# francescofugazzi/3dgsconverter

Hardware: NVIDIA H100
Metric: Msplats/s SOR k=16 (higher is better)
Workload: dtype f32

## Files before the change

### 3dgsconverter_b200/csrc/gsx_abi.cu

```cuda
#include "../../include/gsx.h"

#include "gsx_common.cuh"
#include "gsx_compact.cuh"
#include "gsx_compressed_ply.cuh"
#include "gsx_density.cuh"
#include "gsx_hostcopy.cuh"
#include "gsx_hostrows.cuh"
#include "gsx_kmeans.cuh"
#include "gsx_knn_exact.cuh"
#include "gsx_masks.cuh"
#include "gsx_morton.cuh"
#include "gsx_ply.cuh"
#include "gsx_radix.cuh"
#include "gsx_readers.cuh"
#include "gsx_records.cuh"
#include "gsx_sog.cuh"
#include "gsx_sog_decode.cuh"
#include "gsx_sor.cuh"
#include "gsx_splat_codecs.cuh"

#include <atomic>
#include <math.h>
#include <stdarg.h>
#include <stdio.h>
// ... 166 lines not shown
int gsx_sor_build_from_sorted(const float* spos4_dev, const uint8_t* flags_dev, int64_t n, const float* bmin_host,
                              float cell, void* ws, int64_t ws_bytes, void* stream) {
    SorWs w;
    int rc = carve_grid_checked(ws, ws_bytes, n, w);
    if (rc) return rc;
    GSX_REQUIRE(cell > 0.f, GSX_ERR_ARG, "sor: cell size must be > 0");
    return sor_build_from_sorted((const float4*)spos4_dev, flags_dev, n, bmin_host, cell, w, (cudaStream_t)stream);
}

int gsx_sor_mean_dists_range(int64_t n, int64_t q_begin, int64_t q_end, int32_t k, int32_t hash_mode,
                             const float* bmin_host, float cell, void* ws, int64_t ws_bytes, float* final_means_dev,
                             unsigned long long* stats_dev, void* stream) {
    SorWs w;
    int rc = carve_grid_checked(ws, ws_bytes, n, w);
    if (rc) return rc;
    return sor_mean_dists(w, q_begin, q_end, 1, 0, k, hash_mode, bmin_host, cell, final_means_dev, stats_dev,
                          (cudaStream_t)stream);
}

int gsx_sor_mean_dists_strided(int64_t n, int32_t stride, int32_t phase, int32_t k, int32_t hash_mode,
                               const float* bmin_host, float cell, void* ws, int64_t ws_bytes, float* final_means_dev,
                               unsigned long long* stats_dev, void* stream) {
    SorWs w;
    int rc = carve_grid_checked(ws, ws_bytes, n, w);
    if (rc) return rc;
    return sor_mean_dists(w, 0, n, stride, phase, k, hash_mode, bmin_host, cell, final_means_dev, stats_dev,
                          (cudaStream_t)stream);
}

int gsx_sor_mean_dists(int64_t n, int32_t k, int32_t hash_mode, const float* bmin_host, float cell, void* ws,
                       int64_t ws_bytes, float* final_means_dev, unsigned long long* stats_dev, void* stream) {
    return gsx_sor_mean_dists_range(n, 0, n, k, hash_mode, bmin_host, cell, ws, ws_bytes, final_means_dev, stats_dev,
                                    stream);
}

int64_t gsx_mean_std_workspace_bytes(int64_t n) { return (int64_t)mean_std_ws_bytes(n); }

int gsx_mean_std_f32(const float* a_dev, int64_t n, float* out_dev, void* ws, int64_t ws_bytes, void* stream) {
    return mean_std_f32(a_dev, n, out_dev, ws, (size_t)ws_bytes, (cudaStream_t)stream);
}

int64_t gsx_pairwise_slots(int64_t n) { return pairwise_slots(n); }

int gsx_pairwise_leaves_dist(const float* a_local_dev, int64_t base, int64_t n_local, int64_t n_global, int32_t sq,
                             const float* meanstd_dev, const float* halo_dev, const int64_t* bases_dev, int32_t world,
                             float* slot_dev, void* stream) {
    return pairwise_leaves_dist(a_local_dev, base, n_local, n_global, sq, meanstd_dev, halo_dev,
                                (const long long*)bases_dev, world, slot_dev, (cudaStream_t)stream);
}

int gsx_pairwise_finish(float* slot_dev, int64_t n_global, int32_t sq, float* meanstd_dev, void* stream) {
    GSX_REQUIRE(n_global >= 1, GSX_ERR_ARG, "pairwise_finish: n must be >= 1");
    return pairwise_finish(slot_dev, n_global, sq, meanstd_dev, (cudaStream_t)stream);
}

int gsx_threshold_mask(const float* a_dev, int64_t n, const float* meanstd_dev, float threshold_factor,
                       uint8_t* mask_dev, void* stream) {
    return threshold_mask(a_dev, n, meanstd_dev, threshold_factor, mask_dev, (cudaStream_t)stream);
}

int gsx_sor_filter_device(const float* xyz_dev, int64_t n, int32_t k, float threshold_factor, int32_t hash_mode,
                          uint8_t* mask_dev, float* means_dev, void* ws, int64_t ws_bytes, void* stream) {
    cudaStream_t st = (cudaStream_t)stream;
    SorWs w;
    int rc = carve_checked(ws, ws_bytes, n, w);
    if (rc) return rc;
// ... 419 lines not shown
```

### 3dgsconverter_b200/csrc/gsx_sor.cu

```cuda
#include "gsx_common.cuh"
#include "gsx_sor.cuh"

#include "gsx_radix.cuh"
#include <math.h>

namespace gsx {

#define GSX_D2LIM_BITS 0x60ad78ebu
#define GSX_FULL 0xffffffffu

constexpr int kCellCodeBits = 15;
constexpr float kCellCodeScale = (float)(1 << (kCellCodeBits / 3));
constexpr float kCellCodeMax = kCellCodeScale - 1.f;
constexpr int kSmallBucket = 64;
constexpr int kQueryBatch = 16;
constexpr int kMergeThreshold = 9;
constexpr int kKnnMinBlocks = 8;
constexpr int kFlatSupers = 8;
const char* sor_build_info() {
    return "knn=r02c;epi_smem=1;first_sort=1;query_batch=16;minblocks=8;merge_threshold=9;small_bucket=64;"
           "flat_supers=8;knn16=0;tma=0;i32=1;cell_order=hilbert15";
}


SorWs sor_carve(void* ws, int64_t ws_bytes, int64_t n, size_t sort_ws_bytes) {
    SorWs w;
    Carver c(ws, (size_t)ws_bytes);
    int64_t nchunk = (n + 31) / 32, nsuper = (nchunk + 31) / 32;
    w.n = n;
    w.spos = c.take<float4>(n);
    w.tab_se = c.take<int2>(n);
    w.tab_box = c.take<float4>(2 * n);
    w.startbits = c.take<uint32_t>(nchunk);
    w.cellbits = c.take<uint32_t>(nchunk);
    w.bigbits = c.take<uint32_t>(nchunk);
    w.startlist = c.take<uint32_t>(n / 8 + 1024);
    w.caabb = c.take<float4>(2 * nchunk);
    w.saabb = c.take<float4>(2 * nsuper);
    w.partial = c.take<float>(6 * 1024);
    w.minmax = c.take<float>(8);
    w.counters = c.take<unsigned int>(64);
    w.stats = c.take<unsigned long long>(8);
    w.meanstd = c.take<float>(8);
    w.ms_bytes = mean_std_ws_bytes(n);
    w.ms_ws = c.take<char>(w.ms_bytes);
    w.grid_total = align_up(c.off, 256);
    w.keys0 = c.take<uint64_t>(n);
    w.keys1 = c.take<uint64_t>(n);
    w.sort_ws_bytes = sort_ws_bytes;
    w.sort_ws = c.take<char>(sort_ws_bytes);
    w.total = align_up(c.off, 256);
    w.ok = c.ok();
    w.grid_ok = w.grid_total <= (size_t)(ws_bytes > 0 ? ws_bytes : 0);
// ... 729 lines not shown
    const unsigned tail_blocks = (sl.capacity + 255) / 256;
    k_sor_bucket_tail<<<tail_blocks, 256, 0, st>>>(w.spos, flags, n, bmin[0], bmin[1], bmin[2], cell, M64, w.tab_se,
                                                   w.tab_box, w.bigbits, sl);
    GSX_KERNEL_CHECK();
    k_sor_big_buckets<<<sm_count() * 8, 256, 0, st>>>(w.bigbits, w.startbits, w.spos, w.caabb, n, bmin[0], bmin[1], bmin[2],
                                                      cell, M64, w.tab_se, w.tab_box, sl);
    GSX_KERNEL_CHECK();
    const int resident = sm_count() * 2;
    k_sor_finish_gated<<<resident, 1024, 0, st>>>(w.spos, n, bmin[0], bmin[1], bmin[2], cell, M64, w.tab_se, w.startbits,
                                                  w.cellbits, w.caabb, w.saabb, sl.count + 1);
    GSX_KERNEL_CHECK();
    k_sor_bucket_boxes_gated<<<resident * 4, 256, 0, st>>>(w.startbits, w.spos, w.caabb, w.tab_se, n, bmin[0], bmin[1],
                                                           bmin[2], cell, M64, w.tab_box, sl.count + 1);
    GSX_KERNEL_CHECK();
    return GSX_OK;
}


__device__ __forceinline__ uint32_t probe_hash(int nx, int ny, int nz, uint32_t n, uint64_t M, int mode) {
    if (mode == GSX_HASH_MODE_I32WRAP) {
        int32_t h = (int32_t)((uint32_t)nx * 73856093u) ^ (int32_t)((uint32_t)ny * 19349663u) ^
                    (int32_t)((uint32_t)nz * 83492791u);
        uint32_t a = h < 0 ? (uint32_t)(-(int64_t)h) : (uint32_t)h;
        uint32_t r = fastmod_u32(a, M, n);
        return h < 0 ? (r ? n - r : 0u) : r;
    } else {
        int64_t h = ((int64_t)nx * 73856093LL) ^ ((int64_t)ny * 19349663LL) ^ ((int64_t)nz * 83492791LL);
        int64_t r = h % (int64_t)n;
        if (r < 0) r += n;
        return (uint32_t)r;
    }
}

__device__ __forceinline__ float box_lb(const float4* __restrict__ aabb, int64_t id, float qx, float qy, float qz) {
    float4 a = __ldg(aabb + 2 * id), b = __ldg(aabb + 2 * id + 1);
    float dx = fmaxf(fmaxf(__fsub_rn(a.x, qx), __fsub_rn(qx, a.w)), 0.f);
    float dy = fmaxf(fmaxf(__fsub_rn(a.y, qy), __fsub_rn(qy, b.x)), 0.f);
    float dz = fmaxf(fmaxf(__fsub_rn(a.z, qz), __fsub_rn(qz, b.y)), 0.f);
    return __fadd_rn(__fadd_rn(__fmul_rn(dx, dx), __fmul_rn(dy, dy)), __fmul_rn(dz, dz));
}

__device__ __forceinline__ float cmpx(float v, int j, bool take_min) {
    float o = __shfl_xor_sync(GSX_FULL, v, j);
    return take_min ? fminf(v, o) : fmaxf(v, o);
}

__device__ __forceinline__ float warp_sort32(float v, int lane) {
#pragma unroll
    for (int k = 2; k <= 32; k <<= 1) {
#pragma unroll
        for (int j = k >> 1; j > 0; j >>= 1) v = cmpx(v, j, ((lane & k) == 0) == ((lane & j) == 0));
    }
    return v;
}

template <int NREG>
struct TopK {
    float v0, v1;
    float tau;
    int K;
    __device__ __forceinline__ void init(int k) {
        K = k;
        v0 = v1 = tau = __uint_as_float(GSX_D2LIM_BITS);
    }
    __device__ __forceinline__ void refresh_tau() {
        tau = (NREG == 2 && K > 32) ? __shfl_sync(GSX_FULL, v1, K - 33) : __shfl_sync(GSX_FULL, v0, K - 1);
    }
    __device__ __forceinline__ void insert(float x, int lane) {
        float up0 = __shfl_up_sync(GSX_FULL, v0, 1);
        if (NREG == 2) {
            float top0 = __shfl_sync(GSX_FULL, v0, 31);
            float up1 = __shfl_up_sync(GSX_FULL, v1, 1);
            if (lane == 0) up1 = top0;
            if (v1 > x) v1 = fmaxf(up1, x);
        }
        if (lane == 0) up0 = 0.f;
        if (v0 > x) v0 = fmaxf(up0, x);
        refresh_tau();
    }
    __device__ __forceinline__ void merge32(float nv, int lane) {
        nv = warp_sort32(nv, lane);
        if (__all_sync(GSX_FULL, v0 == __uint_as_float(GSX_D2LIM_BITS))) {
            v0 = nv;
            refresh_tau();
            return;
        }
        float r = __shfl_sync(GSX_FULL, nv, 31 - lane);
        float m = fminf(v0, r);
#pragma unroll
        for (int j = 16; j > 0; j >>= 1) m = cmpx(m, j, (lane & j) == 0);
        v0 = m;
        refresh_tau();
    }
};

typedef int pos_t;

template <int NREG, bool STATS>
__device__ __forceinline__ void scan32(const float4* __restrict__ spos, pos_t j, bool valid, float qx, float qy,
                                       float qz, TopK<NREG>& tk, int lane, unsigned long long& n_scanned) {
    float d2 = INFINITY;
    if (valid) {
        float4 c = __ldg(spos + j);
        float ax = __fsub_rn(qx, c.x), ay = __fsub_rn(qy, c.y), az = __fsub_rn(qz, c.z);
        d2 = __fadd_rn(__fadd_rn(__fmul_rn(ax, ax), __fmul_rn(ay, ay)), __fmul_rn(az, az));
    }
    if (STATS) n_scanned += __popc(__ballot_sync(GSX_FULL, valid));
    bool pass = valid && d2 > 1.0e-12f && d2 < tk.tau;
    unsigned m = __ballot_sync(GSX_FULL, pass);
    if (NREG == 1 && __popc(m) >= kMergeThreshold) {
        tk.merge32(pass ? d2 : __uint_as_float(GSX_D2LIM_BITS), lane);
        return;
    }
    while (m) {
        int src = __ffs(m) - 1;
        m &= m - 1;
        float x = __shfl_sync(GSX_FULL, d2, src);
        if (x < tk.tau) tk.insert(x, lane);
    }
}

template <int NREG, bool STATS, int ES>
__global__ void __launch_bounds__(256, kKnnMinBlocks)
    k_sor_knn(const float4* __restrict__ spos, const int2* __restrict__ tab_se, const float4* __restrict__ tab_box,
              const uint32_t* __restrict__ cellbits, const float4* __restrict__ caabb,
              const float4* __restrict__ saabb, float* __restrict__ final_means, unsigned int* __restrict__ work,
              int64_t q_begin, int64_t q_end, int q_stride, int q_phase, int K, int hash_mode, float bx, float by,
              float bz, float cell,
              uint32_t n, uint64_t M, unsigned long long* __restrict__ stats) {
    const int lane = lane_id();
    unsigned long long st_visits = 0, st_scanned = 0, st_boxes = 0, st_queries = 0;
    static_assert(ES >= 0 && ES <= 33, "a row holds at most the 32 ranks of one register + the row number");
    extern __shared__ float s_epi[];
    float* const epi = s_epi + (threadIdx.x >> 5) * (kQueryBatch * (ES > 0 ? ES : 1));
    const int pdx = lane / 9 - 1, pdy = (lane / 3) % 3 - 1, pdz = lane % 3 - 1;

    for (;;) {
        unsigned int b0 = 0;
        if (lane == 0) b0 = atomicAdd(work, (unsigned)kQueryBatch);
        b0 = __shfl_sync(GSX_FULL, b0, 0);
        int64_t qb = q_begin + ((int64_t)(b0 / kQueryBatch) * q_stride + q_phase) * kQueryBatch;
        if (qb >= q_end) break;
        int64_t qe = qb + kQueryBatch < q_end ? qb + kQueryBatch : q_end;
        const uint32_t cellword = __ldg(cellbits + (qb >> 5));
        int ps = 0, pc = 0;
        float blx = 0.f, bly = 0.f, blz = 0.f, bhx = 0.f, bhy = 0.f, bhz = 0.f;
        const pos_t qb_p = (pos_t)qb, qe_p = (pos_t)qe;
#pragma unroll 1
        for (pos_t i = qb_p; i < qe_p; ++i) {
            const float4 q = __ldg(spos + i);
            const uint32_t w_i = (i >> 5) == (qb_p >> 5) ? cellword : __ldg(cellbits + (i >> 5));
            if (i == qb_p || ((w_i >> (i & 31)) & 1u)) {
                const int gx = (int)floorf(__fdiv_rn(__fsub_rn(q.x, bx), cell));
                const int gy = (int)floorf(__fdiv_rn(__fsub_rn(q.y, by), cell));
                const int gz = (int)floorf(__fdiv_rn(__fsub_rn(q.z, bz), cell));
                ps = 0, pc = 0;
                if (lane < 27) {
                    uint32_t h = probe_hash(gx + pdx, gy + pdy, gz + pdz, n, M, hash_mode);
                    const int2 se = __ldg(tab_se + h);
                    ps = se.x;
                    pc = se.y - se.x;
                    if (pc > 0) {
                        const float4 b0 = __ldg(tab_box + 2 * (size_t)h), b1 = __ldg(tab_box + 2 * (size_t)h + 1);
                        blx = b0.x, bly = b0.y, blz = b0.z, bhx = b1.x, bhy = b1.y, bhz = b1.z;
                    }
                }
            }
            if (STATS) {
                int tot = pc;
#pragma unroll
                for (int o = 16; o > 0; o >>= 1) tot += __shfl_xor_sync(GSX_FULL, tot, o);
                st_visits += (unsigned long long)tot;
                st_queries += 1;
            }
            TopK<NREG> tk;
            tk.init(K);

            unsigned pkey = 0xffffffffu;
            if (pc > 0) {
                float dx = fmaxf(fmaxf(__fsub_rn(blx, q.x), __fsub_rn(q.x, bhx)), 0.f);
                float dy = fmaxf(fmaxf(__fsub_rn(bly, q.y), __fsub_rn(q.y, bhy)), 0.f);
                float dz = fmaxf(fmaxf(__fsub_rn(blz, q.z), __fsub_rn(q.z, bhz)), 0.f);
                pkey = __float_as_uint(__fadd_rn(__fadd_rn(__fmul_rn(dx, dx), __fmul_rn(dy, dy)), __fmul_rn(dz, dz)));
            }

            int skip_chunk = -1;
            {
                int s13 = __shfl_sync(GSX_FULL, ps, 13), c13 = __shfl_sync(GSX_FULL, pc, 13);
                if (c13 > kSmallBucket && i >= s13 && i < (pos_t)s13 + c13) {
                    skip_chunk = (int)(i >> 5);
                    const pos_t j = ((pos_t)skip_chunk << 5) + lane;
                    scan32<NREG, STATS>(spos, j, j >= s13 && j < (pos_t)s13 + c13, q.x, q.y, q.z, tk, lane,
                                        st_scanned);
                }
            }

#pragma unroll 1
            for (;;) {
                const unsigned mp = __reduce_min_sync(GSX_FULL, pkey);
                if (mp == 0xffffffffu || !(__uint_as_float(mp) < tk.tau)) break;
                const int p = __ffs(__ballot_sync(GSX_FULL, pkey == mp)) - 1;
                if (lane == p) pkey = 0xffffffffu;
                const int s = __shfl_sync(GSX_FULL, ps, p), c = __shfl_sync(GSX_FULL, pc, p);
                const pos_t e = (pos_t)s + c;
                if (c <= kSmallBucket) {
#pragma unroll 1
                    for (pos_t base = s; base < e; base += 32)
                        scan32<NREG, STATS>(spos, base + lane, base + lane < e, q.x, q.y, q.z, tk, lane, st_scanned);
                    continue;
                }
                const int skip = p == 13 ? skip_chunk : -1;
                const int fc = s >> 5, lc = (int)((e - 1) >> 5);
                const int fs = fc >> 5, ls = lc >> 5;
                auto chunk_group = [&](const int cbase) {
                    const int cid = cbase + lane;
                    const bool cv = cid >= fc && cid <= lc && cid != skip;
                    unsigned ckey = 0xffffffffu;
                    if (cv) {
                        float lb = box_lb(caabb, cid, q.x, q.y, q.z);
                        if (lb < tk.tau) ckey = __float_as_uint(lb);
                    }
                    if (STATS) st_boxes += __popc(__ballot_sync(GSX_FULL, cv));
                    for (;;) {
                        unsigned mc = __reduce_min_sync(GSX_FULL, ckey);
                        if (mc == 0xffffffffu || !(__uint_as_float(mc) < tk.tau)) break;
                        int srcc = __ffs(__ballot_sync(GSX_FULL, ckey == mc)) - 1;
                        if (lane == srcc) ckey = 0xffffffffu;
                        const pos_t j = ((pos_t)(cbase + srcc) << 5) + lane;
                        scan32<NREG, STATS>(spos, j, j >= s && j < e, q.x, q.y, q.z, tk, lane, st_scanned);
                    }
                };
                if (ls - fs < kFlatSupers) {
                    for (int cb = fc; cb <= lc; cb += 32) chunk_group(cb);
                    continue;
                }
                for (int sb = fs; sb <= ls; sb += 32) {
                    const int sid = sb + lane;
                    unsigned skey = 0xffffffffu;
                    if (sid <= ls) {
                        float lb = box_lb(saabb, sid, q.x, q.y, q.z);
                        if (lb < tk.tau) skey = __float_as_uint(lb);
                    }
                    if (STATS) st_boxes += __popc(__ballot_sync(GSX_FULL, sid <= ls));
                    for (;;) {
                        unsigned ms = __reduce_min_sync(GSX_FULL, skey);
                        if (ms == 0xffffffffu || !(__uint_as_float(ms) < tk.tau)) break;
                        int srcs = __ffs(__ballot_sync(GSX_FULL, skey == ms)) - 1;
                        if (lane == srcs) skey = 0xffffffffu;
                        chunk_group((sb + srcs) * 32);
                    }
                }
            }

            const float d0 = __fsqrt_rn(tk.v0), d1 = NREG == 2 ? __fsqrt_rn(tk.v1) : 0.f;
            if (ES > 0) {
                float* row = epi + (int)(i - qb_p) * ES;
                if (ES <= 32) {
                    if (lane < ES) row[lane] = lane == ES - 1 ? q.w : d0;
                } else {
                    row[lane] = d0;
                    if (lane == 0) row[ES - 1] = q.w;
                }
                continue;
            }
            int valid = __popc(__ballot_sync(GSX_FULL, lane < K && d0 < 0.9e10f));
            if (NREG == 2) valid += __popc(__ballot_sync(GSX_FULL, lane + 32 < K && d1 < 0.9e10f));
            float sum = 0.f;
            for (int r = 0; r < valid; ++r) {
                float x = (NREG == 2 && r >= 32) ? __shfl_sync(GSX_FULL, d1, r - 32) : __shfl_sync(GSX_FULL, d0, r);
                sum = __fadd_rn(sum, x);
            }
            if (lane == 0) final_means[__float_as_int(q.w)] = valid > 0 ? __fdiv_rn(sum, (float)valid) : 0.f;
        }
        if (ES > 0) {
            __syncwarp();
            if (lane < (int)(qe - qb)) {
                const float* row = epi + lane * ES;
                float sum = 0.f;
                int valid = 0;
                for (int r = 0; r < K; ++r) {
                    const float x = row[r];
                    if (x < 0.9e10f) {
                        sum = __fadd_rn(sum, x);
                        ++valid;
                    }
                }
                final_means[__float_as_int(row[ES - 1])] = valid > 0 ? __fdiv_rn(sum, (float)valid) : 0.f;
            }
            __syncwarp();
        }
    }
    if (STATS && lane == 0) {
        atomicAdd(stats + 0, st_visits);
        atomicAdd(stats + 1, st_scanned);
        atomicAdd(stats + 2, st_boxes);
        atomicAdd(stats + 3, st_queries);
    }
}

__global__ void k_fill_f32(float* p, int64_t n, float v) {
    int64_t i = (int64_t)blockIdx.x * blockDim.x + threadIdx.x;
    if (i < n) p[i] = v;
}

template <int NREG, int ES>
static int launch_knn(SorWs& w, int64_t q_begin, int64_t q_end, int q_stride, int q_phase, int K, int hash_mode,
                      const float* bmin, float cell,
                      float* final_means, unsigned long long* stats, uint64_t M, int64_t want, cudaStream_t st) {
    const auto kernel = stats ? k_sor_knn<NREG, true, ES> : k_sor_knn<NREG, false, ES>;
    int per_sm = 0;
    const size_t smem = (size_t)8 * kQueryBatch * ES * sizeof(float);
    GSX_CUDA_CHECK(cudaOccupancyMaxActiveBlocksPerMultiprocessor(&per_sm, kernel, 256, smem));
    int64_t grid = (int64_t)sm_count() * (per_sm > 0 ? per_sm : 4);
    if (grid > want) grid = want;
    if (grid < 1) grid = 1;
    kernel<<<(int)grid, 256, smem, st>>>(w.spos, w.tab_se, w.tab_box, w.cellbits, w.caabb, w.saabb, final_means, w.counters,
                                         q_begin, q_end, q_stride, q_phase, K, hash_mode, bmin[0], bmin[1], bmin[2], cell,
                                         (uint32_t)w.n, M, stats);
    return GSX_OK;
}

int sor_mean_dists(SorWs& w, int64_t q_begin, int64_t q_end, int q_stride, int q_phase, int k, int hash_mode,
                   const float* bmin, float cell,
                   float* final_means, unsigned long long* stats, cudaStream_t st) {
    GSX_NVTX("gsx::sor_mean_dists(k_sor_knn)");
    int64_t n = w.n;
    GSX_REQUIRE(k >= 1, GSX_ERR_ARG, "sor: k must be >= 1 (got %d)", k);
    GSX_REQUIRE(hash_mode == 0 || hash_mode == 1, GSX_ERR_ARG, "sor: bad hash_mode %d", hash_mode);
    GSX_REQUIRE(q_begin >= 0 && q_end <= n && q_begin <= q_end, GSX_ERR_ARG, "sor: bad query range");
    GSX_REQUIRE(q_stride >= 1 && q_phase >= 0 && q_phase < q_stride, GSX_ERR_ARG, "sor: bad query stride/phase");
    int K = k < 50 ? k : 50;
    if (q_end == q_begin) return GSX_OK;
    if (!(cell > 1e-8f)) {
        GSX_REQUIRE(q_begin == 0 && q_end == n, GSX_ERR_UNSUPPORTED, "sor: degenerate cell with a query range");
        k_fill_f32<<<(int)((n + 255) / 256), 256, 0, st>>>(final_means, n, 0.f);
        GSX_KERNEL_CHECK();
        return GSX_OK;
    }
    GSX_CUDA_CHECK(cudaMemsetAsync(w.counters, 0, sizeof(unsigned int), st));
    uint64_t M = 0xFFFFFFFFFFFFFFFFull / (uint64_t)n + 1ull;
    int64_t nq = (q_end - q_begin + q_stride - 1) / q_stride + kQueryBatch;
    int64_t want = (nq + (int64_t)kQueryBatch * 8 - 1) / ((int64_t)kQueryBatch * 8);
    int rc;
    if (K <= 16)
        rc = launch_knn<1, 17>(w, q_begin, q_end, q_stride, q_phase, K, hash_mode, bmin, cell, final_means, stats, M, want, st);
    else if (K <= 32)
        rc = launch_knn<1, 33>(w, q_begin, q_end, q_stride, q_phase, K, hash_mode, bmin, cell, final_means, stats, M, want, st);
    else
        rc = launch_knn<2, 0>(w, q_begin, q_end, q_stride, q_phase, K, hash_mode, bmin, cell, final_means, stats, M, want, st);
    if (rc) return rc;
    GSX_KERNEL_CHECK();
    return GSX_OK;
}

}
```

### 3dgsconverter_b200/gsx/_abi.py

```python
from __future__ import annotations

import ctypes as C
import os
from pathlib import Path

_PKG = Path(__file__).resolve().parent.parent
LIB_PATH = Path(os.environ.get("GSX_LIB", _PKG / "lib" / "libgsx.so"))


class GsxError(RuntimeError):
    """A libgsx entry point returned a non-zero status."""


if not LIB_PATH.exists():
    raise ImportError(
        f"libgsx.so not found at {LIB_PATH}: build it with `python -c 'import __graft_entry__ as g; g.build()'` "
        "(nvcc, sm_90a).  gsx has no CPU fallback.")

lib = C.CDLL(str(LIB_PATH))

_f32p = C.POINTER(C.c_float)
_vp = C.c_void_p
_i64 = C.c_int64
_i32 = C.c_int32

_SIGS = {
    "gsx_last_error": (C.c_char_p, []),
    "gsx_version": (C.c_int, []),
    "gsx_build_info": (C.c_char_p, []),
    "gsx_device_sm_count": (C.c_int, []),
    "gsx_kernel_launches": (C.c_longlong, []),
    "gsx_sor_workspace_bytes": (_i64, [_i64]),
    "gsx_sor_grid_workspace_bytes": (_i64, [_i64]),
    "gsx_sor_minmax": (C.c_int, [_vp, _i64, _vp, _vp, _i64, _vp]),
    "gsx_sor_cell_size": (C.c_float, [_f32p, _i64]),
    "gsx_sor_build": (C.c_int, [_vp, _i64, _f32p, C.c_float, _vp, _i64, _vp]),
    "gsx_sor_dist_local_run": (C.c_int, [_vp, _i64, _i64, _i64, _i32, _f32p, C.c_float, _vp, _vp, _vp, _i64, _vp]),
    "gsx_sor_dist_merge": (C.c_int, [_vp, _i64, _i64, _i64, _i64, _f32p, C.c_float, _vp, _vp, _vp, _i64, _vp]),
    "gsx_sor_spos_offset": (_i64, [_i64]),
    "gsx_sor_build_from_sorted": (C.c_int, [_vp, _vp, _i64, _f32p, C.c_float, _vp, _i64, _vp]),
    "gsx_sor_mean_dists": (C.c_int, [_i64, _i32, _i32, _f32p, C.c_float, _vp, _i64, _vp, _vp, _vp]),
    "gsx_sor_mean_dists_range": (C.c_int, [_i64, _i64, _i64, _i32, _i32, _f32p, C.c_float, _vp, _i64, _vp, _vp, _vp]),
    "gsx_sor_mean_dists_strided": (C.c_int, [_i64, _i32, _i32, _i32, _i32, _f32p, C.c_float, _vp, _i64, _vp, _vp, _vp]),
    "gsx_sort_pairs_workspace_bytes": (_i64, [_i64]),
    "gsx_sort_pairs": (C.c_int, [_vp, _vp, _i64, _i32, _i32, _vp, _i64, _vp]),
    "gsx_mean_std_workspace_bytes": (_i64, [_i64]),
    "gsx_mean_std_f32": (C.c_int, [_vp, _i64, _vp, _vp, _i64, _vp]),
    "gsx_pairwise_slots": (_i64, [_i64]),
    "gsx_pairwise_leaves_dist": (C.c_int, [_vp, _i64, _i64, _i64, _i32, _vp, _vp, _vp, _i32, _vp, _vp]),
    "gsx_pairwise_finish": (C.c_int, [_vp, _i64, _i32, _vp, _vp]),
    "gsx_threshold_mask": (C.c_int, [_vp, _i64, _vp, C.c_float, _vp, _vp]),
    "gsx_sor_filter_device": (C.c_int, [_vp, _i64, _i32, C.c_float, _i32, _vp, _vp, _vp, _i64, _vp]),
    "gsx_sor_filter_host": (C.c_int, [_vp, _i64, _i32, C.c_float, _i32, _vp, _vp]),
    "gsx_knn_exact_workspace_bytes": (_i64, [_i64]),
    "gsx_knn_exact_mean_dists": (C.c_int, [_vp, _i64, _i32, _vp, _vp, _i64, _vp]),
    "gsx_sor_ckdtree_filter_host": (C.c_int, [_vp, _i64, _i32, C.c_float, _vp, _vp]),
    "gsx_bbox_mask": (C.c_int, [_vp, _i64, _f32p, _vp, _vp]),
    "gsx_alpha_mask": (C.c_int, [_vp, _i64, C.c_double, _vp, _vp]),
    "gsx_alpha_logit_threshold": (C.c_double, [C.c_double]),
    "gsx_compact_workspace_bytes": (_i64, [_i64]),
    "gsx_compact_points": (C.c_int, [_vp, _i64, _vp, _vp, _vp, _vp, _vp, _vp, C.POINTER(_i64), _vp, _i64, _vp]),
    "gsx_density_workspace_bytes": (_i64, [_i64, _i64]),
    "gsx_density_voxel_count": (C.c_int, [_vp, _i64, C.c_float, _i64, _vp, _vp, _i64, C.POINTER(_i64),
                                          C.POINTER(_i64), _vp, _i64, _vp]),
    "gsx_density_member_mask": (C.c_int, [_vp, _i64, C.c_float, _vp, _i64, _vp, _vp, _i64, _vp]),
    "gsx_density_voxel_range": (None, [_f32p, C.c_float, C.POINTER(_i64), C.POINTER(_i64)]),
    "gsx_density_grid_count": (C.c_int, [_vp, _i64, C.c_float, C.POINTER(_i64), C.POINTER(_i64), _vp, _vp, _vp]),
    "gsx_density_grid_dense": (C.c_int, [_vp, C.POINTER(_i64), C.POINTER(_i64), _i64, _vp, _vp, _i64,
                                         C.POINTER(_i64), C.POINTER(_i64), _vp, _i64, _vp]),
    "gsx_lexsort_workspace_bytes": (_i64, [_i64]),
    "gsx_lexsort_zyx": (C.c_int, [_vp, _i64, _vp, _vp, _i64, _vp]),
    "gsx_quantize_to_codebook": (C.c_int, [_vp, _i64, _f32p, _i32, _vp, _vp, _i64, _vp]),
    "gsx_sog_means_minmax": (C.c_int, [_vp, _i64, _i32, C.POINTER(_i32), _vp, _i64, _vp, _vp]),
    "gsx_sog_means": (C.c_int, [_vp, _i64, _i32, _vp, C.POINTER(_i32), _vp, _i64, _vp, _vp, _vp]),
    "gsx_sog_quats": (C.c_int, [_vp, _i64, _i32, _vp, C.POINTER(_i32), _i64, _vp, _vp]),
    "gsx_sog_gather_values": (C.c_int, [_vp, _i64, _i32, _vp, C.POINTER(_i32), _i32, _vp, _i64, _vp, _vp]),
# ... 66 lines not shown
```

### 3dgsconverter_b200/gsx/sor.py

```python
from __future__ import annotations

import ctypes as C
from dataclasses import dataclass

import numpy as np
import torch

from . import _abi
from ._abi import lib, check, HASH_MODES


def _stream():
    return C.c_void_p(torch.cuda.current_stream().cuda_stream)


def _ptr(t):
    return C.c_void_p(t.data_ptr()) if t is not None else C.c_void_p(0)


def default_hash_mode() -> str:
    import os
    return os.environ.get("GSX_SOR_HASH", "i32wrap")


# ... 8 lines not shown
class SorGrid:
    n: int
    ws: torch.Tensor
    bmin: np.ndarray
    cell: float


def workspace(n: int, device) -> torch.Tensor:
    nbytes = lib.gsx_sor_workspace_bytes(n)
    if nbytes <= 0:
        raise _abi.GsxError("gsx_sor_workspace_bytes failed")
    return torch.empty(nbytes, dtype=torch.uint8, device=device)


def build_grid(xyz: torch.Tensor, ws: torch.Tensor | None = None, cell_scale: float = 1.0) -> SorGrid:
    _check_xyz(xyz)
    n = xyz.shape[0]
    if ws is None:
        ws = workspace(n, xyz.device)
    mm_dev = torch.empty(8, dtype=torch.float32, device=xyz.device)
    check(lib.gsx_sor_minmax(_ptr(xyz), n, _ptr(mm_dev), _ptr(ws), ws.numel(), _stream()), "gsx_sor_minmax")
    mm = mm_dev[:6].cpu().numpy()
    cell = float(lib.gsx_sor_cell_size(mm.ctypes.data_as(C.POINTER(C.c_float)), n))
    if cell != cell:
        raise _abi.GsxError("sor: non-finite coordinates")
    if cell_scale != 1.0:
        cell = float(np.float32(cell * cell_scale))
    bmin = mm[:3].copy()
    check(lib.gsx_sor_build(_ptr(xyz), n, bmin.ctypes.data_as(C.POINTER(C.c_float)), cell, _ptr(ws), ws.numel(),
                            _stream()), "gsx_sor_build")
    return SorGrid(n, ws, bmin, cell)


def mean_dists(grid: SorGrid, k: int, hash_mode: str | None = None, out: torch.Tensor | None = None,
               want_stats: bool = False, q_range: tuple[int, int] | None = None):
    mode = HASH_MODES[hash_mode or default_hash_mode()]
    dev = grid.ws.device
    if out is None:
        out = torch.empty(grid.n, dtype=torch.float32, device=dev)
    stats = torch.zeros(4, dtype=torch.int64, device=dev) if want_stats else None
    qb, qe = q_range if q_range is not None else (0, grid.n)
    check(lib.gsx_sor_mean_dists_range(grid.n, qb, qe, int(k), mode, grid.bmin.ctypes.data_as(C.POINTER(C.c_float)),
                                       grid.cell, _ptr(grid.ws), grid.ws.numel(), _ptr(out), _ptr(stats), _stream()),
          "gsx_sor_mean_dists")
    if want_stats:
        v = stats.cpu().numpy()
        return out, dict(visits=int(v[0]), scanned=int(v[1]), box_tests=int(v[2]), queries=int(v[3]))
    return out


def mean_dists_strided(grid: SorGrid, k: int, hash_mode: str | None, out: torch.Tensor, stride: int, phase: int,
                       want_stats: bool = False):
    mode = HASH_MODES[hash_mode or default_hash_mode()]
    stats = torch.zeros(4, dtype=torch.int64, device=out.device) if want_stats else None
    check(lib.gsx_sor_mean_dists_strided(grid.n, int(stride), int(phase), int(k), mode,
                                         grid.bmin.ctypes.data_as(C.POINTER(C.c_float)), grid.cell, _ptr(grid.ws),
                                         grid.ws.numel(), _ptr(out), _ptr(stats), _stream()), "gsx_sor_mean_dists_strided")
    if want_stats:
        v = stats.cpu().numpy()
        return out, dict(visits=int(v[0]), scanned=int(v[1]), box_tests=int(v[2]), queries=int(v[3]))
    return out


def mean_std(a: torch.Tensor) -> torch.Tensor:
    n = a.numel()
    ws = torch.empty(lib.gsx_mean_std_workspace_bytes(n), dtype=torch.uint8, device=a.device)
    out = torch.empty(2, dtype=torch.float32, device=a.device)
    check(lib.gsx_mean_std_f32(_ptr(a), n, _ptr(out), _ptr(ws), ws.numel(), _stream()), "gsx_mean_std_f32")
    return out


def threshold_mask(a: torch.Tensor, meanstd: torch.Tensor, threshold_factor: float) -> torch.Tensor:
    mask = torch.empty(a.numel(), dtype=torch.uint8, device=a.device)
    check(lib.gsx_threshold_mask(_ptr(a), a.numel(), _ptr(meanstd), float(np.float32(threshold_factor)), _ptr(mask),
                                 _stream()), "gsx_threshold_mask")
    return mask.view(torch.bool)


def sor_filter(xyz: torch.Tensor, k: int = 25, threshold_factor: float = 1.0, hash_mode: str | None = None,
               ws: torch.Tensor | None = None, return_means: bool = False):
    _check_xyz(xyz)
    n = xyz.shape[0]
    mode = HASH_MODES[hash_mode or default_hash_mode()]
    if ws is None:
        ws = workspace(n, xyz.device)
    mask = torch.empty(n, dtype=torch.uint8, device=xyz.device)
    means = torch.empty(n, dtype=torch.float32, device=xyz.device) if return_means else None
    check(lib.gsx_sor_filter_device(_ptr(xyz), n, int(k), float(np.float32(threshold_factor)), mode, _ptr(mask),
                                    _ptr(means), _ptr(ws), ws.numel(), _stream()), "gsx_sor_filter_device")
    mask = mask.view(torch.bool)
    return (mask, means) if return_means else mask


# ... 52 lines not shown
```

### include/gsx.h

```cpp
#ifndef GSX_H
#define GSX_H
#include <stdint.h>

#ifdef __cplusplus
extern "C" {
#endif

#define GSX_HASH_I32WRAP 0
#define GSX_HASH_I64 1

const char* gsx_last_error(void);
int gsx_version(void);
const char* gsx_build_info(void);
int gsx_device_sm_count(void);
long long gsx_kernel_launches(void);


int64_t gsx_sor_workspace_bytes(int64_t n);
int64_t gsx_sor_grid_workspace_bytes(int64_t n);

int gsx_sor_minmax(const float* xyz_dev, int64_t n, float* minmax_dev, void* ws, int64_t ws_bytes, void* stream);

float gsx_sor_cell_size(const float* minmax_host, int64_t n);

int gsx_sor_build(const float* xyz_dev, int64_t n, const float* bmin_host, float cell, void* ws, int64_t ws_bytes,
                  void* stream);

int gsx_sor_dist_local_run(const float* xyz_local_dev, int64_t n_local, int64_t idx_base, int64_t n_global,
                           int32_t world, const float* bmin_host, float cell, float* pos4_out_dev,
                           int64_t* cuts_dev, void* ws, int64_t ws_bytes, void* stream);
int gsx_sor_dist_merge(const float* pos4_dev, int64_t m, int64_t n_global, int64_t bucket_lo, int64_t bucket_hi,
                       const float* bmin_host, float cell, float* pos4_sorted_dev,
                       uint8_t* flags_sorted_dev , void* ws, int64_t ws_bytes, void* stream);
int64_t gsx_sor_spos_offset(int64_t n);
int gsx_sor_build_from_sorted(const float* spos4_dev, const uint8_t* flags_dev , int64_t n,
                              const float* bmin_host, float cell, void* ws, int64_t ws_bytes, void* stream);

int gsx_sor_mean_dists(int64_t n, int32_t k, int32_t hash_mode, const float* bmin_host, float cell, void* ws,
                       int64_t ws_bytes, float* final_means_dev, unsigned long long* stats_dev, void* stream);

int gsx_sor_mean_dists_range(int64_t n, int64_t q_begin, int64_t q_end, int32_t k, int32_t hash_mode,
                             const float* bmin_host, float cell, void* ws, int64_t ws_bytes, float* final_means_dev,
                             unsigned long long* stats_dev, void* stream);

int gsx_sor_mean_dists_strided(int64_t n, int32_t stride, int32_t phase, int32_t k, int32_t hash_mode,
                               const float* bmin_host, float cell, void* ws, int64_t ws_bytes, float* final_means_dev,
                               unsigned long long* stats_dev, void* stream);

int64_t gsx_sort_pairs_workspace_bytes(int64_t n);
int gsx_sort_pairs(uint64_t* keys_dev, int32_t* vals_dev, int64_t n, int32_t begin_bit, int32_t end_bit, void* ws,
                   int64_t ws_bytes, void* stream);

int64_t gsx_mean_std_workspace_bytes(int64_t n);
int gsx_mean_std_f32(const float* a_dev, int64_t n, float* out_dev, void* ws, int64_t ws_bytes, void* stream);

int64_t gsx_pairwise_slots(int64_t n);
int gsx_pairwise_leaves_dist(const float* a_local_dev, int64_t base, int64_t n_local, int64_t n_global, int32_t sq,
                             const float* meanstd_dev, const float* halo_dev, const int64_t* bases_dev, int32_t world,
                             float* slot_dev, void* stream);
int gsx_pairwise_finish(float* slot_dev, int64_t n_global, int32_t sq, float* meanstd_dev, void* stream);

int gsx_threshold_mask(const float* a_dev, int64_t n, const float* meanstd_dev, float threshold_factor,
                       uint8_t* mask_dev, void* stream);

int gsx_sor_filter_device(const float* xyz_dev, int64_t n, int32_t k, float threshold_factor, int32_t hash_mode,
                          uint8_t* mask_dev, float* means_dev, void* ws, int64_t ws_bytes, void* stream);

int gsx_sor_filter_host(const float* xyz_host, int64_t n, int32_t k, float threshold_factor, int32_t hash_mode,
                        uint8_t* mask_host, float* means_host);

int64_t gsx_knn_exact_workspace_bytes(int64_t n);
int gsx_knn_exact_mean_dists(const float* xyz_dev, int64_t n, int32_t k, float* means_dev, void* ws, int64_t ws_bytes,
                             void* stream);
int gsx_sor_ckdtree_filter_host(const float* xyz_host, int64_t n, int32_t k, float threshold_factor, uint8_t* mask_host,
                                float* means_host);

int gsx_bbox_mask(const float* xyz_dev, int64_t n, const float* lohi_host , uint8_t* mask_dev, void* stream);
int gsx_alpha_mask(const float* opacity_dev, int64_t n, double logit_thresh, uint8_t* mask_dev, void* stream);
double gsx_alpha_logit_threshold(double min_opacity_u8);

// ... 130 lines not shown
```

Before: 1226.

## Pack lane index into kNN traversal keys and defer tau refresh

Traversal keys for probes, supers and chunks now carry the lane index in their low 5 bits, so one reduce_min picks the winning lane without a separate ballot/ffs, and the sentinel check folds into the lower-bound comparison. scan32 returns early when no candidate passes, drops the per-insert tau recheck, and refreshes tau once after the insertion loop instead of after every insert. The center-cell shuffles are hoisted out of the per-query path. Per-lane query counters are added behind the STATS template flag. Truncating the bound's low mantissa bits slightly loosens pruning, and skipping per-insert tau updates may insert candidates that would otherwise have been rejected.

```diff
diff --git a/3dgsconverter_b200/csrc/gsx_abi.cu b/3dgsconverter_b200/csrc/gsx_abi.cu
--- a/3dgsconverter_b200/csrc/gsx_abi.cu
+++ b/3dgsconverter_b200/csrc/gsx_abi.cu
@@ -222,6 +222,17 @@
                        int64_t ws_bytes, float* final_means_dev, unsigned long long* stats_dev, void* stream) {
     return gsx_sor_mean_dists_range(n, 0, n, k, hash_mode, bmin_host, cell, ws, ws_bytes, final_means_dev, stats_dev,
                                     stream);
+}
+
+int gsx_sor_query_counters(int64_t n, void* ws, int64_t ws_bytes, unsigned long long* out8_host, void* stream) {
+    SorWs w;
+    int rc = carve_grid_checked(ws, ws_bytes, n, w);
+    if (rc) return rc;
+    GSX_REQUIRE(out8_host != nullptr, GSX_ERR_ARG, "sor: null counter buffer");
+    GSX_CUDA_CHECK(cudaMemcpyAsync(out8_host, w.stats, 8 * sizeof(unsigned long long), cudaMemcpyDeviceToHost,
+                                   (cudaStream_t)stream));
+    GSX_CUDA_CHECK(cudaStreamSynchronize((cudaStream_t)stream));
+    return GSX_OK;
 }
 
 int64_t gsx_mean_std_workspace_bytes(int64_t n) { return (int64_t)mean_std_ws_bytes(n); }
diff --git a/3dgsconverter_b200/csrc/gsx_sor.cu b/3dgsconverter_b200/csrc/gsx_sor.cu
--- a/3dgsconverter_b200/csrc/gsx_sor.cu
+++ b/3dgsconverter_b200/csrc/gsx_sor.cu
@@ -18,7 +18,7 @@
 constexpr int kKnnMinBlocks = 8;
 constexpr int kFlatSupers = 8;
 const char* sor_build_info() {
-    return "knn=r02c;epi_smem=1;first_sort=1;query_batch=16;minblocks=8;merge_threshold=9;small_bucket=64;"
+    return "knn=r03a;epi_smem=1;first_sort=1;query_batch=16;minblocks=8;merge_threshold=9;small_bucket=64;"
            "flat_supers=8;knn16=0;tma=0;i32=1;cell_order=hilbert15";
 }
 
@@ -814,6 +814,10 @@
     }
 }
 
+constexpr unsigned kKeyNone = 0xffffffffu;
+__device__ __forceinline__ unsigned knn_key(float lb, int lane) { return (__float_as_uint(lb) & ~31u) | (unsigned)lane; }
+__device__ __forceinline__ float knn_key_lb(unsigned key) { return __uint_as_float(key & ~31u); }
+
 __device__ __forceinline__ float box_lb(const float4* __restrict__ aabb, int64_t id, float qx, float qy, float qz) {
     float4 a = __ldg(aabb + 2 * id), b = __ldg(aabb + 2 * id + 1);
     float dx = fmaxf(fmaxf(__fsub_rn(a.x, qx), __fsub_rn(qx, a.w)), 0.f);
@@ -858,14 +862,13 @@
         }
         if (lane == 0) up0 = 0.f;
         if (v0 > x) v0 = fmaxf(up0, x);
-        refresh_tau();
-    }
-    __device__ __forceinline__ void merge32(float nv, int lane) {
+    }
+    __device__ __forceinline__ bool merge32(float nv, int lane) {
         nv = warp_sort32(nv, lane);
         if (__all_sync(GSX_FULL, v0 == __uint_as_float(GSX_D2LIM_BITS))) {
             v0 = nv;
             refresh_tau();
-            return;
+            return true;
         }
         float r = __shfl_sync(GSX_FULL, nv, 31 - lane);
         float m = fminf(v0, r);
@@ -873,14 +876,32 @@
         for (int j = 16; j > 0; j >>= 1) m = cmpx(m, j, (lane & j) == 0);
         v0 = m;
         refresh_tau();
+        return false;
     }
 };
+
+enum KnnCounter {
+    kCntInserts,
+    kCntMergesFirst,
+    kCntMergesFull,
+    kCntProbeVisits,
+    kCntSuperVisits,
+    kCntChunkGroups,
+    kCntChunkVisits,
+    kCntScanSteps,
+    kCntCount
+};
+template <bool STATS>
+__device__ __forceinline__ void knn_count(unsigned long long& cnt, int lane, KnnCounter c) {
+    if (STATS && lane == (int)c) ++cnt;
+}
 
 typedef int pos_t;
 
 template <int NREG, bool STATS>
 __device__ __forceinline__ void scan32(const float4* __restrict__ spos, pos_t j, bool valid, float qx, float qy,
-                                       float qz, TopK<NREG>& tk, int lane, unsigned long long& n_scanned) {
+                                       float qz, TopK<NREG>& tk, int lane, unsigned long long& n_scanned,
+                                       unsigned long long& cnt) {
     float d2 = INFINITY;
     if (valid) {
         float4 c = __ldg(spos + j);
@@ -888,18 +909,22 @@
         d2 = __fadd_rn(__fadd_rn(__fmul_rn(ax, ax), __fmul_rn(ay, ay)), __fmul_rn(az, az));
     }
     if (STATS) n_scanned += __popc(__ballot_sync(GSX_FULL, valid));
+    knn_count<STATS>(cnt, lane, kCntScanSteps);
     bool pass = valid && d2 > 1.0e-12f && d2 < tk.tau;
     unsigned m = __ballot_sync(GSX_FULL, pass);
+    if (m == 0u) return;
     if (NREG == 1 && __popc(m) >= kMergeThreshold) {
-        tk.merge32(pass ? d2 : __uint_as_float(GSX_D2LIM_BITS), lane);
+        const bool first = tk.merge32(pass ? d2 : __uint_as_float(GSX_D2LIM_BITS), lane);
+        knn_count<STATS>(cnt, lane, first ? kCntMergesFirst : kCntMergesFull);
         return;
     }
     while (m) {
         int src = __ffs(m) - 1;
         m &= m - 1;
-        float x = __shfl_sync(GSX_FULL, d2, src);
-        if (x < tk.tau) tk.insert(x, lane);
-    }
+        tk.insert(__shfl_sync(GSX_FULL, d2, src), lane);
+        knn_count<STATS>(cnt, lane, kCntInserts);
+    }
+    tk.refresh_tau();
 }
 
 template <int NREG, bool STATS, int ES>
@@ -909,9 +934,11 @@
               const float4* __restrict__ saabb, float* __restrict__ final_means, unsigned int* __restrict__ work,
               int64_t q_begin, int64_t q_end, int q_stride, int q_phase, int K, int hash_mode, float bx, float by,
               float bz, float cell,
-              uint32_t n, uint64_t M, unsigned long long* __restrict__ stats) {
+              uint32_t n, uint64_t M, unsigned long long* __restrict__ stats,
+              unsigned long long* __restrict__ query_counters) {
     const int lane = lane_id();
     unsigned long long st_visits = 0, st_scanned = 0, st_boxes = 0, st_queries = 0;
+    unsigned long long st_cnt = 0;
     static_assert(ES >= 0 && ES <= 33, "a row holds at most the 32 ranks of one register + the row number");
     extern __shared__ float s_epi[];
     float* const epi = s_epi + (threadIdx.x >> 5) * (kQueryBatch * (ES > 0 ? ES : 1));
@@ -926,6 +953,7 @@
         int64_t qe = qb + kQueryBatch < q_end ? qb + kQueryBatch : q_end;
         const uint32_t cellword = __ldg(cellbits + (qb >> 5));
         int ps = 0, pc = 0;
+        int s13 = 0, c13 = 0;
         float blx = 0.f, bly = 0.f, blz = 0.f, bhx = 0.f, bhy = 0.f, bhz = 0.f;
         const pos_t qb_p = (pos_t)qb, qe_p = (pos_t)qe;
 #pragma unroll 1
@@ -947,6 +975,7 @@
                         blx = b0.x, bly = b0.y, blz = b0.z, bhx = b1.x, bhy = b1.y, bhz = b1.z;
                     }
                 }
+                s13 = __shfl_sync(GSX_FULL, ps, 13), c13 = __shfl_sync(GSX_FULL, pc, 13);
             }
             if (STATS) {
                 int tot = pc;
@@ -958,37 +987,36 @@
             TopK<NREG> tk;
             tk.init(K);
 
-            unsigned pkey = 0xffffffffu;
+            unsigned pkey = kKeyNone;
             if (pc > 0) {
                 float dx = fmaxf(fmaxf(__fsub_rn(blx, q.x), __fsub_rn(q.x, bhx)), 0.f);
                 float dy = fmaxf(fmaxf(__fsub_rn(bly, q.y), __fsub_rn(q.y, bhy)), 0.f);
                 float dz = fmaxf(fmaxf(__fsub_rn(blz, q.z), __fsub_rn(q.z, bhz)), 0.f);
-                pkey = __float_as_uint(__fadd_rn(__fadd_rn(__fmul_rn(dx, dx), __fmul_rn(dy, dy)), __fmul_rn(dz, dz)));
+                pkey = knn_key(__fadd_rn(__fadd_rn(__fmul_rn(dx, dx), __fmul_rn(dy, dy)), __fmul_rn(dz, dz)), lane);
             }
 
             int skip_chunk = -1;
-            {
-                int s13 = __shfl_sync(GSX_FULL, ps, 13), c13 = __shfl_sync(GSX_FULL, pc, 13);
-                if (c13 > kSmallBucket && i >= s13 && i < (pos_t)s13 + c13) {
-                    skip_chunk = (int)(i >> 5);
-                    const pos_t j = ((pos_t)skip_chunk << 5) + lane;
-                    scan32<NREG, STATS>(spos, j, j >= s13 && j < (pos_t)s13 + c13, q.x, q.y, q.z, tk, lane,
-                                        st_scanned);
-                }
+            if (c13 > kSmallBucket && i >= s13 && i < (pos_t)s13 + c13) {
+                skip_chunk = (int)(i >> 5);
+                const pos_t j = ((pos_t)skip_chunk << 5) + lane;
+                scan32<NREG, STATS>(spos, j, j >= s13 && j < (pos_t)s13 + c13, q.x, q.y, q.z, tk, lane, st_scanned,
+                                    st_cnt);
             }
 
 #pragma unroll 1
             for (;;) {
                 const unsigned mp = __reduce_min_sync(GSX_FULL, pkey);
-                if (mp == 0xffffffffu || !(__uint_as_float(mp) < tk.tau)) break;
-                const int p = __ffs(__ballot_sync(GSX_FULL, pkey == mp)) - 1;
-                if (lane == p) pkey = 0xffffffffu;
+                if (!(knn_key_lb(mp) < tk.tau)) break;
+                const int p = (int)(mp & 31u);
+                if (lane == p) pkey = kKeyNone;
+                knn_count<STATS>(st_cnt, lane, kCntProbeVisits);
                 const int s = __shfl_sync(GSX_FULL, ps, p), c = __shfl_sync(GSX_FULL, pc, p);
                 const pos_t e = (pos_t)s + c;
                 if (c <= kSmallBucket) {
 #pragma unroll 1
                     for (pos_t base = s; base < e; base += 32)
-                        scan32<NREG, STATS>(spos, base + lane, base + lane < e, q.x, q.y, q.z, tk, lane, st_scanned);
+                        scan32<NREG, STATS>(spos, base + lane, base + lane < e, q.x, q.y, q.z, tk, lane, st_scanned,
+                                            st_cnt);
                     continue;
                 }
                 const int skip = p == 13 ? skip_chunk : -1;
@@ -997,19 +1025,21 @@
                 auto chunk_group = [&](const int cbase) {
                     const int cid = cbase + lane;
                     const bool cv = cid >= fc && cid <= lc && cid != skip;
-                    unsigned ckey = 0xffffffffu;
+                    unsigned ckey = kKeyNone;
                     if (cv) {
                         float lb = box_lb(caabb, cid, q.x, q.y, q.z);
-                        if (lb < tk.tau) ckey = __float_as_uint(lb);
+                        if (lb < tk.tau) ckey = knn_key(lb, lane);
                     }
                     if (STATS) st_boxes += __popc(__ballot_sync(GSX_FULL, cv));
+                    knn_count<STATS>(st_cnt, lane, kCntChunkGroups);
                     for (;;) {
-                        unsigned mc = __reduce_min_sync(GSX_FULL, ckey);
-                        if (mc == 0xffffffffu || !(__uint_as_float(mc) < tk.tau)) break;
-                        int srcc = __ffs(__ballot_sync(GSX_FULL, ckey == mc)) - 1;
-                        if (lane == srcc) ckey = 0xffffffffu;
+                        const unsigned mc = __reduce_min_sync(GSX_FULL, ckey);
+                        if (!(knn_key_lb(mc) < tk.tau)) break;
+                        const int srcc = (int)(mc & 31u);
+                        if (lane == srcc) ckey = kKeyNone;
+                        knn_count<STATS>(st_cnt, lane, kCntChunkVisits);
                         const pos_t j = ((pos_t)(cbase + srcc) << 5) + lane;
-                        scan32<NREG, STATS>(spos, j, j >= s && j < e, q.x, q.y, q.z, tk, lane, st_scanned);
+                        scan32<NREG, STATS>(spos, j, j >= s && j < e, q.x, q.y, q.z, tk, lane, st_scanned, st_cnt);
                     }
                 };
                 if (ls - fs < kFlatSupers) {
@@ -1018,17 +1048,18 @@
                 }
                 for (int sb = fs; sb <= ls; sb += 32) {
                     const int sid = sb + lane;
-                    unsigned skey = 0xffffffffu;
+                    unsigned skey = kKeyNone;
                     if (sid <= ls) {
                         float lb = box_lb(saabb, sid, q.x, q.y, q.z);
-                        if (lb < tk.tau) skey = __float_as_uint(lb);
+                        if (lb < tk.tau) skey = knn_key(lb, lane);
                     }
                     if (STATS) st_boxes += __popc(__ballot_sync(GSX_FULL, sid <= ls));
                     for (;;) {
-                        unsigned ms = __reduce_min_sync(GSX_FULL, skey);
-                        if (ms == 0xffffffffu || !(__uint_as_float(ms) < tk.tau)) break;
-                        int srcs = __ffs(__ballot_sync(GSX_FULL, skey == ms)) - 1;
-                        if (lane == srcs) skey = 0xffffffffu;
+                        const unsigned ms = __reduce_min_sync(GSX_FULL, skey);
+                        if (!(knn_key_lb(ms) < tk.tau)) break;
+                        const int srcs = (int)(ms & 31u);
+                        if (lane == srcs) skey = kKeyNone;
+                        knn_count<STATS>(st_cnt, lane, kCntSuperVisits);
                         chunk_group((sb + srcs) * 32);
                     }
                 }
@@ -1078,6 +1109,7 @@
         atomicAdd(stats + 2, st_boxes);
         atomicAdd(stats + 3, st_queries);
     }
+    if (STATS && lane < kCntCount) atomicAdd(query_counters + lane, st_cnt);
 }
 
 __global__ void k_fill_f32(float* p, int64_t n, float v) {
@@ -1098,7 +1130,7 @@
     if (grid < 1) grid = 1;
     kernel<<<(int)grid, 256, smem, st>>>(w.spos, w.tab_se, w.tab_box, w.cellbits, w.caabb, w.saabb, final_means, w.counters,
                                          q_begin, q_end, q_stride, q_phase, K, hash_mode, bmin[0], bmin[1], bmin[2], cell,
-                                         (uint32_t)w.n, M, stats);
+                                         (uint32_t)w.n, M, stats, w.stats);
     return GSX_OK;
 }
 
@@ -1112,6 +1144,7 @@
     GSX_REQUIRE(q_begin >= 0 && q_end <= n && q_begin <= q_end, GSX_ERR_ARG, "sor: bad query range");
     GSX_REQUIRE(q_stride >= 1 && q_phase >= 0 && q_phase < q_stride, GSX_ERR_ARG, "sor: bad query stride/phase");
     int K = k < 50 ? k : 50;
+    if (stats) GSX_CUDA_CHECK(cudaMemsetAsync(w.stats, 0, kCntCount * sizeof(unsigned long long), st));
     if (q_end == q_begin) return GSX_OK;
     if (!(cell > 1e-8f)) {
         GSX_REQUIRE(q_begin == 0 && q_end == n, GSX_ERR_UNSUPPORTED, "sor: degenerate cell with a query range");
diff --git a/3dgsconverter_b200/gsx/_abi.py b/3dgsconverter_b200/gsx/_abi.py
--- a/3dgsconverter_b200/gsx/_abi.py
+++ b/3dgsconverter_b200/gsx/_abi.py
@@ -42,6 +42,7 @@
     "gsx_sor_mean_dists": (C.c_int, [_i64, _i32, _i32, _f32p, C.c_float, _vp, _i64, _vp, _vp, _vp]),
     "gsx_sor_mean_dists_range": (C.c_int, [_i64, _i64, _i64, _i32, _i32, _f32p, C.c_float, _vp, _i64, _vp, _vp, _vp]),
     "gsx_sor_mean_dists_strided": (C.c_int, [_i64, _i32, _i32, _i32, _i32, _f32p, C.c_float, _vp, _i64, _vp, _vp, _vp]),
+    "gsx_sor_query_counters": (C.c_int, [_i64, _vp, _i64, _vp, _vp]),
     "gsx_sort_pairs_workspace_bytes": (_i64, [_i64]),
     "gsx_sort_pairs": (C.c_int, [_vp, _vp, _i64, _i32, _i32, _vp, _i64, _vp]),
     "gsx_mean_std_workspace_bytes": (_i64, [_i64]),
diff --git a/3dgsconverter_b200/gsx/sor.py b/3dgsconverter_b200/gsx/sor.py
--- a/3dgsconverter_b200/gsx/sor.py
+++ b/3dgsconverter_b200/gsx/sor.py
@@ -64,6 +64,19 @@
     return SorGrid(n, ws, bmin, cell)
 
 
+QUERY_COUNTERS = ("inserts", "merges_first", "merges_full", "probe_visits", "super_visits", "chunk_groups",
+                  "chunk_visits", "scan_steps")
+
+
+def _stats_dict(grid: SorGrid, stats: torch.Tensor) -> dict:
+    v = stats.cpu().numpy()
+    c = (C.c_ulonglong * 8)()
+    check(lib.gsx_sor_query_counters(grid.n, _ptr(grid.ws), grid.ws.numel(), C.cast(c, C.c_void_p), _stream()),
+          "gsx_sor_query_counters")
+    return dict(visits=int(v[0]), scanned=int(v[1]), box_tests=int(v[2]), queries=int(v[3]),
+                **{name: int(c[i]) for i, name in enumerate(QUERY_COUNTERS)})
+
+
 def mean_dists(grid: SorGrid, k: int, hash_mode: str | None = None, out: torch.Tensor | None = None,
                want_stats: bool = False, q_range: tuple[int, int] | None = None):
     mode = HASH_MODES[hash_mode or default_hash_mode()]
@@ -76,8 +89,7 @@
                                        grid.cell, _ptr(grid.ws), grid.ws.numel(), _ptr(out), _ptr(stats), _stream()),
           "gsx_sor_mean_dists")
     if want_stats:
-        v = stats.cpu().numpy()
-        return out, dict(visits=int(v[0]), scanned=int(v[1]), box_tests=int(v[2]), queries=int(v[3]))
+        return out, _stats_dict(grid, stats)
     return out
 
 
@@ -89,8 +101,7 @@
                                          grid.bmin.ctypes.data_as(C.POINTER(C.c_float)), grid.cell, _ptr(grid.ws),
                                          grid.ws.numel(), _ptr(out), _ptr(stats), _stream()), "gsx_sor_mean_dists_strided")
     if want_stats:
-        v = stats.cpu().numpy()
-        return out, dict(visits=int(v[0]), scanned=int(v[1]), box_tests=int(v[2]), queries=int(v[3]))
+        return out, _stats_dict(grid, stats)
     return out
 
 
diff --git a/include/gsx.h b/include/gsx.h
--- a/include/gsx.h
+++ b/include/gsx.h
@@ -46,6 +46,8 @@
 int gsx_sor_mean_dists_strided(int64_t n, int32_t stride, int32_t phase, int32_t k, int32_t hash_mode,
                                const float* bmin_host, float cell, void* ws, int64_t ws_bytes, float* final_means_dev,
                                unsigned long long* stats_dev, void* stream);
+
+int gsx_sor_query_counters(int64_t n, void* ws, int64_t ws_bytes, unsigned long long* out8_host, void* stream);
 
 int64_t gsx_sort_pairs_workspace_bytes(int64_t n);
 int gsx_sort_pairs(uint64_t* keys_dev, int32_t* vals_dev, int64_t n, int32_t begin_bit, int32_t end_bit, void* ws,
```

After: 1285, median of 6. 4.8% higher.
